# apcamargo/genomad

Hardware: AMD Instinct MI355X
Metric: 6 kbp windows classified/sec (higher is better)
Workload: dtype f16x3tk (conv2 read from a 137 GB table of all 14-mers in HBM - x2[t] is a function of the bases t-10 .. t+3 -, head A's pair products from an (entry, 9-mer) table, head A's y @ w_v rows from a 9-mer table, all exact f32; conv3 by Toom-Cook F(3,6) with split-f16 MFMA, 3 products per operand pair, f3

## Files before the change

genomad_amd/csrc/gnn_api.hip:

```cpp
#include <algorithm>
#include <map>
#include <mutex>
#include <cstdio>
#include <cmath>
#include <cstdlib>
#include <cstring>

#include "gnn_common.h"

namespace gnn {

static thread_local std::string g_last_error;
void set_error(const std::string& msg) { g_last_error = msg; }

bool debug_switch(const char* name) {
    static std::mutex mu;
    static std::map<std::string, bool> seen;
    std::lock_guard<std::mutex> lock(mu);
    auto it = seen.find(name);
    if (it != seen.end()) return it->second;
    const bool on = std::getenv(name) != nullptr;
    if (on)
        std::fprintf(stderr, "libgenomad_nn_hip: debug switch %s is set: NOT the production path (ordering or arithmetic may differ)\n", name);
    seen[name] = on;
    return on;
}

struct ProfScope {
    gnn_ctx* ctx;
    int id;
    hipEvent_t a = nullptr, b = nullptr;
    ProfScope(gnn_ctx* c, int kid) : ctx(c), id(kid) {
        if (!ctx->profile) return;
        auto take = [&]() {
            hipEvent_t e = nullptr;
            if (!ctx->event_pool.empty()) {
                e = ctx->event_pool.back();
                ctx->event_pool.pop_back();
            } else if (hipEventCreate(&e) != hipSuccess) {
                e = nullptr;
            }
            return e;
        };
        a = take();
        b = take();
        if (a) (void)hipEventRecord(a, ctx->stream);
    }
    ~ProfScope() {
        if (!ctx->profile || !a || !b) return;
        (void)hipEventRecord(b, ctx->stream);
        ctx->prof[id].pending.emplace_back(a, b);
    }
};

static void free_ws(Workspace& ws) { ws = Workspace(); }

constexpr size_t WS_BYTES_PER_WINDOW = ((size_t)2 * NPAIR + 2 * NP + (size_t)2 * POOLED * C + 4 * POOLED + FEAT) * sizeof(float);
constexpr int64_t MIN_CHUNK = 256;

static int ensure_ws(gnn_ctx* ctx, Workspace& ws, int64_t chunk, int64_t x_chunk) {
    if (ws.chunk < chunk || ws.x_chunk < x_chunk) {
        if (ctx->stream2) GNN_HIP(hipStreamSynchronize(ctx->stream2));
        ctx->back_pending[0] = ctx->back_pending[1] = false;
    }
    if (ws.chunk < chunk) {
        GNN_HIP(hipStreamSynchronize(ctx->stream));
        int rc = ws.mp.reserve((size_t)chunk * 2 * NPAIR);
        if (!rc) rc = ws.m.reserve((size_t)chunk * 2 * NP);
        if (!rc) rc = ws.yp.reserve((size_t)chunk * 2 * POOLED * C);
        if (!rc) rc = ws.logits.reserve((size_t)chunk * 2 * POOLED);
        if (!rc) rc = ws.alpha.reserve((size_t)chunk * 2 * POOLED);
        if (!rc) rc = ws.feat.reserve((size_t)chunk * FEAT);
        if (rc) {
            free_ws(ws);
            return rc;
        }
        ws.chunk = chunk;
    }
    if (ws.x_chunk < x_chunk) {
        GNN_HIP(hipStreamSynchronize(ctx->stream));
        ws.x_chunk = 0;
        for (DevBuf<float>& x : ws.x) x.reset();
        ws.tokens.reset();
        int rc = GNN_OK;
        for (DevBuf<float>& x : ws.x)
            if (!rc) rc = x.reserve((size_t)x_chunk * T * C);
        if (!rc) rc = ws.tokens.reserve((size_t)x_chunk * T);
        if (rc) {
            free_ws(ws);
            return rc;
        }
        ws.x_chunk = x_chunk;
    }
    return GNN_OK;
}

int flush_backend(gnn_ctx* ctx) {
    for (int i = 0; i < 2; ++i)
        if (ctx->back_pending[i]) {
            GNN_HIP(hipStreamWaitEvent(ctx->stream, ctx->ev_back[i], 0));
            ctx->back_pending[i] = false;
        }
    return GNN_OK;
}

int finish_pending(gnn_ctx* ctx) {
    if (ctx->back_pending[0] || ctx->back_pending[1]) {
        GNN_HIP(hipStreamSynchronize(ctx->stream2));
        ctx->back_pending[0] = ctx->back_pending[1] = false;
    }
    return GNN_OK;
}

static int check_ctx(gnn_ctx* ctx, bool flush = true) {
    if (!ctx) {
        set_error("ctx is NULL");
        return GNN_ERR_ARG;
    }
    GNN_HIP(hipSetDevice(ctx->device));
    if (!flush) return GNN_OK;
    static const bool event_wait = debug_switch("GNN_ASYNC_EVENT_WAIT");
// ... 141 lines not shown
    }
    bool overlap = allow_overlap && !f32 && ((chunk_overlap && n > chunk) || defer_last || pending);
    if (overlap && ctx->alt_failed_chunk > 0 && chunk >= ctx->alt_failed_chunk && ctx->ws_alt.chunk < chunk) {
        if ((rc = flush_backend(ctx))) return rc;
        overlap = false;
    }
    if (overlap && (rc = ensure_ws(ctx, ctx->ws_alt, chunk, 0)) == GNN_ERR_NOMEM) {
        std::fprintf(stderr, "libgenomad_nn_hip: no device memory for the second workspace of %lld windows: asynchronous calls run in order "
                     "(back end not overlapped) from here on\n", (long long)chunk);
        ctx->alt_failed_chunk = chunk;
        if ((rc = flush_backend(ctx))) return rc;
        overlap = false;
    } else if (rc) {
        return rc;
    }
    if (overlap) {
        if (!ctx->stream2) {
            GNN_HIP(hipStreamCreateWithFlags(&ctx->stream2, hipStreamNonBlocking));
            for (int i = 0; i < 2; ++i) {
                GNN_HIP(hipEventCreateWithFlags(&ctx->ev_front[i], hipEventDisableTiming));
                GNN_HIP(hipEventCreateWithFlags(&ctx->ev_back[i], hipEventDisableTiming));
            }
        }
    }
    struct StreamGuard {
        gnn_ctx* c;
        hipStream_t main;
        ~StreamGuard() { c->stream = main; }
    } guard{ctx, ctx->stream};
    for (int64_t a = 0; a < n; a += chunk) {
        const int64_t m = std::min(chunk, n - a);
        const uint8_t* b = bases_dev + a * W;
        if (!f32 && (reinterpret_cast<uintptr_t>(b) & 3u)) {
            if (ctx->align_buf.capacity() < (size_t)m * W) {
                GNN_HIP(hipStreamSynchronize(guard.main));
                if ((rc = ctx->align_buf.reserve((size_t)chunk * W))) return rc;
            }
            GNN_HIP(hipMemcpyAsync(ctx->align_buf, b, (size_t)m * W, hipMemcpyDeviceToDevice, guard.main));
            b = ctx->align_buf;
        }
        const int buf = ctx->buf_cur;
        if (overlap && ctx->back_pending[buf]) {
            GNN_HIP(hipStreamWaitEvent(guard.main, ctx->ev_back[buf], 0));
            ctx->back_pending[buf] = false;
        }
        static const bool poison = debug_switch("GNN_DEBUG_POISON");
        if (poison) {
            const Workspace& ws = ctx->ws;
            const size_t mm = (size_t)std::min<int64_t>(m, ws.chunk);
            auto fill = [&](float* p, size_t per_window) -> int {
                if (p && mm) GNN_HIP(hipMemsetAsync(p, 0xFF, mm * per_window * sizeof(float), guard.main));
                return GNN_OK;
            };
            if ((rc = fill(ws.mp, 2 * NPAIR)) || (rc = fill(ws.m, 2 * NP)) || (rc = fill(ws.yp, (size_t)2 * POOLED * C)) ||
                (rc = fill(ws.logits, 2 * POOLED)) || (rc = fill(ws.alpha, 2 * POOLED)) || (rc = fill(ws.feat, FEAT)))
                return rc;
            if (emb_dev)
                GNN_HIP(hipMemsetAsync(static_cast<uint8_t*>(emb_dev) + (size_t)a * HID * emb_elem_bytes(emb_dtype), 0xFF,
                                       (size_t)m * HID * emb_elem_bytes(emb_dtype), guard.main));
        }
        if (f32) {
            ProfScope ps(ctx, GNN_K_F32_FRONT);
            if ((rc = launch_front_f32(ctx, b, m))) return rc;
        } else {
            ProfScope ps(ctx, GNN_K_FUSED);
            rc = precision == GNN_PREC_F16X3TK ? launch_front_tk(ctx, b, m)
                 : precision == GNN_PREC_F16X3TC ? launch_front_tc(ctx, b, m)
                 : precision == GNN_PREC_F16C6 ? launch_front_c6(ctx, b, m)
                                               : launch_front_x3(ctx, b, m, precision);
            if (rc) return rc;
        }
        if (overlap) {
            GNN_HIP(hipEventRecord(ctx->ev_front[buf], guard.main));
            ctx->stream = ctx->stream2;
            GNN_HIP(hipStreamWaitEvent(ctx->stream2, ctx->ev_front[buf], 0));
        }
        {
            ProfScope ps(ctx, GNN_K_BACKEND);
            void* emb = emb_dev ? static_cast<uint8_t*>(emb_dev) + (size_t)a * HID * emb_elem_bytes(emb_dtype) : nullptr;
            rc = launch_backend(ctx, m, (precision == GNN_PREC_F16X3TC || precision == GNN_PREC_F16X3TK) ? GNN_PREC_F16X3 : precision,
                                scores_dev + a * GNN_CLASSES, emb, emb_dtype);
        }
        if (overlap) {
            if (!rc) {
                GNN_HIP(hipEventRecord(ctx->ev_back[buf], ctx->stream2));
                ctx->back_pending[buf] = true;
            }
            ctx->stream = guard.main;
            std::swap(ctx->ws, ctx->ws_alt);
            ctx->buf_cur ^= 1;
        }
        if (rc) return rc;
    }
    return defer_last ? GNN_OK : flush_backend(ctx);
}

}

using namespace gnn;

extern "C" {

const char* gnn_last_error(void) { return g_last_error.c_str(); }

int gnn_version(void) { return 300; }

int gnn_debug_pack_c6(const float* w, int k, int n, uint32_t* out, size_t out_words, size_t* need_words) {
// ... 500 lines not shown
    const size_t row = (size_t)HID * emb_elem_bytes(emb_dtype);
    if ((rc = ensure_stage(ctx, slab))) return rc;
    if (ctx->stage_emb.capacity() * sizeof(float) < (size_t)slab * row) {
        GNN_HIP(hipStreamSynchronize(ctx->stream));
        if ((rc = ctx->stage_emb.reserve((size_t)slab * HID))) return rc;
    }
    for (int64_t a0 = 0; a0 < n && !rc; a0 += slab) {
        const int64_t m = std::min(slab, n - a0);
        rc = stage_upload(ctx, bases_host + a0 * W, (size_t)m * W);
        if (!rc) rc = classify_chunks(ctx, ctx->stage_bases, m, precision, ctx->stage_scores, false, ctx->stage_emb, emb_dtype);
        if (!rc) {
            if (scores_host)
                GNN_HIP(hipMemcpyAsync(ctx->stage_scores_host, ctx->stage_scores, (size_t)m * GNN_CLASSES * sizeof(float),
                                       hipMemcpyDeviceToHost, ctx->stream));
            GNN_HIP(hipMemcpyAsync(static_cast<uint8_t*>(emb_host) + (size_t)a0 * row, ctx->stage_emb, (size_t)m * row,
                                   hipMemcpyDeviceToHost, ctx->stream));
            GNN_HIP(hipStreamSynchronize(ctx->stream));
            if (scores_host)
                std::memcpy(scores_host + a0 * GNN_CLASSES, ctx->stage_scores_host, (size_t)m * GNN_CLASSES * sizeof(float));
        }
    }
    return rc;
}

int gnn_classify(gnn_ctx* ctx, const uint8_t* bases_host, int64_t n, int precision, float* scores_host) {
    return gnn_debug_forward(ctx, bases_host, n, precision, scores_host, nullptr);
}

int gnn_debug_forward(gnn_ctx* ctx, const uint8_t* bases_host, int64_t n, int precision,
                      float* scores_host, const gnn_taps* taps) {
    int rc = check_ctx(ctx);
    if (rc) return rc;
    if (n < 0 || (n > 0 && (!bases_host || !scores_host))) {
        set_error("bad argument to gnn_classify");
        return GNN_ERR_ARG;
    }
    if (n == 0) return GNN_OK;
    if (taps) {
        const int64_t lim = precision == GNN_PREC_F32 ? ctx->chunk_f32 : ctx->chunk_fused;
        if (n > lim) {
            set_error("gnn_debug_forward with taps: n_windows exceeds one chunk (" + std::to_string(lim) + ")");
            return GNN_ERR_ARG;
        }
        if ((taps->x1 || taps->x2 || taps->x3) && precision != GNN_PREC_F32) {
            set_error("x1/x2/x3 taps exist only on the f32 path (the fused path keeps them in LDS)");
            return GNN_ERR_ARG;
        }
    }
    const int64_t slab = std::min<int64_t>(n, STAGE_MAX_WINDOWS);
    if ((rc = ensure_stage(ctx, slab))) return rc;
    for (int64_t a0 = 0; a0 < n && !rc; a0 += slab) {
        const int64_t m = std::min(slab, n - a0);
        rc = stage_upload(ctx, bases_host + a0 * W, (size_t)m * W);
        if (!rc) rc = classify_chunks(ctx, ctx->stage_bases, m, precision, ctx->stage_scores);
        if (!rc) {
            GNN_HIP(hipMemcpyAsync(ctx->stage_scores_host, ctx->stage_scores, (size_t)m * GNN_CLASSES * sizeof(float),
                                   hipMemcpyDeviceToHost, ctx->stream));
            GNN_HIP(hipStreamSynchronize(ctx->stream));
            std::memcpy(scores_host + a0 * GNN_CLASSES, ctx->stage_scores_host, (size_t)m * GNN_CLASSES * sizeof(float));
        }
    }
    if (!rc && taps && precision != GNN_PREC_F32 && n > ctx->chunk_fused) {
        set_error("gnn_debug_forward with taps: the launch size was reduced to " + std::to_string(ctx->chunk_fused) +
                  " windows for lack of device memory; the taps of " + std::to_string(n) + " windows do not fit one launch");
        return GNN_ERR_STATE;
    }
    if (!rc && taps) {
        const Workspace& ws = ctx->ws;
        auto out = [&](float* dst, const float* src, size_t count) {
            if (dst && !rc) rc = gnn_memcpy_d2h(ctx, dst, src, count * sizeof(float));
        };
        out(taps->x1, ws.x[0], (size_t)n * T * C);
        out(taps->x2, ws.x[1], (size_t)n * T * C);
        out(taps->x3, ws.x[2], (size_t)n * T * C);
        out(taps->feat, ws.feat, (size_t)n * FEAT);
        auto out2 = [&](float* dst_a, float* dst_b, const float* src, size_t per) {
            if ((!dst_a && !dst_b) || rc) return;
            std::vector<float> tmp((size_t)n * 2 * per);
            rc = gnn_memcpy_d2h(ctx, tmp.data(), src, tmp.size() * sizeof(float));
            if (rc) return;
            for (int64_t i = 0; i < n; ++i) {
                if (dst_a) std::memcpy(dst_a + i * per, tmp.data() + (i * 2 + 0) * per, per * sizeof(float));
                if (dst_b) std::memcpy(dst_b + i * per, tmp.data() + (i * 2 + 1) * per, per * sizeof(float));
            }
        };
        out2(taps->yp_a, taps->yp_b, ws.yp, (size_t)POOLED * C);
        out2(taps->alpha_a, taps->alpha_b, ws.alpha, (size_t)POOLED);
        out2(taps->m_a, taps->m_b, ws.m, (size_t)NP);
    }
    return rc;
}

static int upload_spans(gnn_ctx* ctx, const int64_t* starts_host, const int32_t* lens_host, int64_t n,
                        DevBuf<int64_t>& starts_dev, DevBuf<int32_t>& lens_dev) {
    for (int64_t i = 0; i < n; ++i)
        if (starts_host[i] < 0 || lens_host[i] < 0 || lens_host[i] > W) {
            set_error("span " + std::to_string(i) + " has a negative start or a length outside [0, 6000]");
            return GNN_ERR_ARG;
        }
    int rc = starts_dev.reserve((size_t)n);
    if (!rc) rc = lens_dev.reserve((size_t)n);
    if (!rc) rc = gnn_memcpy_h2d(ctx, starts_dev, starts_host, (size_t)n * sizeof(int64_t));
    if (!rc) rc = gnn_memcpy_h2d(ctx, lens_dev, lens_host, (size_t)n * sizeof(int32_t));
    return rc;
}

int gnn_span_byte_count(gnn_ctx* ctx, const uint8_t* seq_dev, const int64_t* starts_host, const int32_t* lens_host,
// ... 130 lines not shown
```

genomad_amd/csrc/gnn_backend.hip:

```cpp
#include <cstdlib>

#include "gnn_common.h"

namespace gnn {

__global__ __launch_bounds__(256) void m_kernel(const float* __restrict__ mp, const float* __restrict__ w_bias0,
                                                const float* __restrict__ w_bias1,
                                                const int32_t* __restrict__ slot0,
                                                const int32_t* __restrict__ slot1, float* __restrict__ m) {
    __shared__ float s[NPAIR];
    const int wi = blockIdx.x, h = blockIdx.y;
    const float* w_bias = h ? w_bias1 : w_bias0;
    const int32_t* slot = h ? slot1 : slot0;
    const float4* src = reinterpret_cast<const float4*>(mp + ((size_t)wi * 2 + h) * NPAIR);
    for (int i = threadIdx.x; i < NPAIR / 4; i += 256) reinterpret_cast<float4*>(s)[i] = src[i];
    __syncthreads();
    for (int p = threadIdx.x; p < NP; p += 256) {
        const int4 sl = reinterpret_cast<const int4*>(slot)[p];
        m[((size_t)wi * 2 + h) * NP + p] = w_bias[p] + s[sl.x] + s[sl.y] + s[sl.z] + s[sl.w];
    }
}

constexpr int LW = 64, LQ = 128, LK = 16;

__global__ __launch_bounds__(256) void logits_kernel(const float* __restrict__ m,
                                                     const float* __restrict__ w_qk0,
                                                     const float* __restrict__ w_qk1, int n,
                                                     float* __restrict__ logits) {
    __shared__ __attribute__((aligned(16))) float ms[LK][LW + 4];
    __shared__ __attribute__((aligned(16))) float qs[LK][LQ];
    const int h = blockIdx.z;
    const float* w_qk = h ? w_qk1 : w_qk0;
    const int w0 = blockIdx.y * LW;
    const int q0 = blockIdx.x * LQ;
    const int tw = threadIdx.x >> 4;
    const int tq = threadIdx.x & 15;
    float acc[4][8];
#pragma unroll
    for (int i = 0; i < 4; ++i)
#pragma unroll
        for (int k = 0; k < 8; ++k) acc[i][k] = 0.f;
    for (int p0 = 0; p0 < NP; p0 += LK) {
        {
            const int w = threadIdx.x >> 2, pq = (threadIdx.x & 3) * 4;
            float4 v = make_float4(0.f, 0.f, 0.f, 0.f);
            if (w0 + w < n && p0 + pq < NP)
                v = *reinterpret_cast<const float4*>(m + ((size_t)(w0 + w) * 2 + h) * NP + p0 + pq);
            ms[pq][w] = v.x;
            ms[pq + 1][w] = v.y;
            ms[pq + 2][w] = v.z;
            ms[pq + 3][w] = v.w;
        }
        for (int i = threadIdx.x; i < LK * LQ; i += 256) {
            const int q = i % LQ, p = i / LQ;
            qs[p][q] = (p0 + p < NP && q0 + q < POOLED) ? w_qk[(size_t)(p0 + p) * POOLED + q0 + q] : 0.f;
        }
        __syncthreads();
#pragma unroll 4
        for (int p = 0; p < LK; ++p) {
            const float4 a = *reinterpret_cast<const float4*>(&ms[p][tw * 4]);
            const float4 b0 = *reinterpret_cast<const float4*>(&qs[p][tq * 4]);
            const float4 b1 = *reinterpret_cast<const float4*>(&qs[p][64 + tq * 4]);
            const float av[4] = {a.x, a.y, a.z, a.w};
            const float bv[8] = {b0.x, b0.y, b0.z, b0.w, b1.x, b1.y, b1.z, b1.w};
#pragma unroll
            for (int i = 0; i < 4; ++i)
#pragma unroll
                for (int k = 0; k < 8; ++k) acc[i][k] = fmaf(av[i], bv[k], acc[i][k]);
        }
        __syncthreads();
    }
#pragma unroll
    for (int i = 0; i < 4; ++i) {
        const int w = w0 + tw * 4 + i;
        if (w >= n) continue;
#pragma unroll
        for (int k = 0; k < 8; ++k) {
            const int q = q0 + (k >> 2) * 64 + tq * 4 + (k & 3);
            if (q < POOLED) logits[((size_t)w * 2 + h) * POOLED + q] = acc[i][k];
        }
    }
}

typedef __bf16 bf16x8 __attribute__((ext_vector_type(8)));
typedef float f32x16 __attribute__((ext_vector_type(16)));

struct QkA {
    float4 v[2][2];
};
struct QkB {
    uint4 v[2][2];
};

__device__ __forceinline__ void qk_load(QkA& a, QkB& b, const float* __restrict__ mrow0, const float* __restrict__ mrow1,
                                        const uint4* __restrict__ bfrag, int ks, int lane) {
    const int k = ks * 16 + (lane >> 5) * 8;
    const float* rows[2] = {mrow0, mrow1};
#pragma unroll
    for (int mb = 0; mb < 2; ++mb) {
        if (k + 8 <= NP) {
            a.v[mb][0] = *reinterpret_cast<const float4*>(rows[mb] + k);
            a.v[mb][1] = *reinterpret_cast<const float4*>(rows[mb] + k + 4);
        } else {
            float t[8];
#pragma unroll
            for (int e = 0; e < 8; ++e) t[e] = k + e < NP ? rows[mb][k + e] : 0.f;
            a.v[mb][0] = make_float4(t[0], t[1], t[2], t[3]);
            a.v[mb][1] = make_float4(t[4], t[5], t[6], t[7]);
        }
    }
    const uint4* bp = bfrag + (size_t)ks * (QK_NBLK * 2 * 64);
#pragma unroll
    for (int nb = 0; nb < 2; ++nb) {
        b.v[nb][0] = bp[nb * 2 * 64];
        b.v[nb][1] = bp[nb * 2 * 64 + 64];
    }
}

template <int PASSES, bool F16>
__device__ __forceinline__ void qk_mfma(const QkA& a, const QkB& b, f32x16 (&acc)[2][2]) {
    typedef float f32x8 __attribute__((ext_vector_type(8)));
    typedef _Float16 f16x8q __attribute__((ext_vector_type(8)));
#pragma unroll
    for (int mb = 0; mb < 2; ++mb) {
        const f32x8 x = {a.v[mb][0].x, a.v[mb][0].y, a.v[mb][0].z, a.v[mb][0].w,
                         a.v[mb][1].x, a.v[mb][1].y, a.v[mb][1].z, a.v[mb][1].w};
        if constexpr (F16) {
            const f16x8q ah = __builtin_convertvector(x, f16x8q);
            const f16x8q al = __builtin_convertvector(x - __builtin_convertvector(ah, f32x8), f16x8q);
#pragma unroll
            for (int nb = 0; nb < 2; ++nb) {
                const f16x8q bh = __builtin_bit_cast(f16x8q, b.v[nb][0]);
                if constexpr (PASSES == 3) {
                    const f16x8q bl = __builtin_bit_cast(f16x8q, b.v[nb][1]);
                    acc[mb][nb] = __builtin_amdgcn_mfma_f32_32x32x16_f16(ah, bl, acc[mb][nb], 0, 0, 0);
                    acc[mb][nb] = __builtin_amdgcn_mfma_f32_32x32x16_f16(al, bh, acc[mb][nb], 0, 0, 0);
                }
                acc[mb][nb] = __builtin_amdgcn_mfma_f32_32x32x16_f16(ah, bh, acc[mb][nb], 0, 0, 0);
            }
        } else {
            const bf16x8 ah = __builtin_convertvector(x, bf16x8);
            const bf16x8 al = __builtin_convertvector(x - __builtin_convertvector(ah, f32x8), bf16x8);
#pragma unroll
            for (int nb = 0; nb < 2; ++nb) {
                const bf16x8 bh = __builtin_bit_cast(bf16x8, b.v[nb][0]);
                if constexpr (PASSES == 3) {
                    const bf16x8 bl = __builtin_bit_cast(bf16x8, b.v[nb][1]);
                    acc[mb][nb] = __builtin_amdgcn_mfma_f32_32x32x16_bf16(ah, bl, acc[mb][nb], 0, 0, 0);
                    acc[mb][nb] = __builtin_amdgcn_mfma_f32_32x32x16_bf16(al, bh, acc[mb][nb], 0, 0, 0);
                }
                acc[mb][nb] = __builtin_amdgcn_mfma_f32_32x32x16_bf16(ah, bh, acc[mb][nb], 0, 0, 0);
            }
        }
    }
}

template <int PASSES, bool F16 = false>
__global__ __launch_bounds__(256) void logits_mfma_kernel(const float* __restrict__ m, const uint4* __restrict__ frag0,
                                                          const uint4* __restrict__ frag1, int n,
                                                          float* __restrict__ logits) {
    const int lane = threadIdx.x & 63, wave = threadIdx.x >> 6;
    const int h = blockIdx.z;
    const int w0 = blockIdx.y * 64;
    const int nb0 = blockIdx.x * 8 + wave * 2;
    const uint4* bfrag = (h ? frag1 : frag0) + (size_t)nb0 * 2 * 64 + lane;
    const float* mrow0 = m + ((size_t)min(w0 + (lane & 31), n - 1) * 2 + h) * NP;
    const float* mrow1 = m + ((size_t)min(w0 + 32 + (lane & 31), n - 1) * 2 + h) * NP;
    f32x16 acc[2][2];
#pragma unroll
    for (int i = 0; i < 2; ++i)
#pragma unroll
        for (int j = 0; j < 2; ++j)
#pragma unroll
            for (int r = 0; r < 16; ++r) acc[i][j][r] = 0.f;
    QkA a0, a1;
    QkB b0, b1;
    qk_load(a0, b0, mrow0, mrow1, bfrag, 0, lane);
#pragma unroll 1
    for (int ks = 0; ks < QK_KSTEPS; ks += 2) {
        qk_load(a1, b1, mrow0, mrow1, bfrag, ks + 1, lane);
        qk_mfma<PASSES, F16>(a0, b0, acc);
        qk_load(a0, b0, mrow0, mrow1, bfrag, min(ks + 2, QK_KSTEPS - 1), lane);
        qk_mfma<PASSES, F16>(a1, b1, acc);
    }
#pragma unroll
    for (int mb = 0; mb < 2; ++mb)
#pragma unroll
        for (int r = 0; r < 16; ++r) {
            const int w = w0 + mb * 32 + (r & 3) + 8 * (r >> 2) + 4 * (lane >> 5);
            if (w >= n) continue;
#pragma unroll
            for (int nb = 0; nb < 2; ++nb) {
                const int q = (nb0 + nb) * 32 + (lane & 31);
                if (q < POOLED) logits[((size_t)w * 2 + h) * POOLED + q] = acc[mb][nb][r];
            }
        }
}

__global__ __launch_bounds__(256) void attn_kernel(const float* __restrict__ logits,
                                                   const float* __restrict__ yp,
                                                   float* __restrict__ alpha_out,
                                                   float* __restrict__ feat) {
    __shared__ float a[POOLED + 3];
    __shared__ float red[256];
    const int wi = blockIdx.x, h = blockIdx.y;
    const float* lg = logits + ((size_t)wi * 2 + h) * POOLED;
    float mx = -INFINITY;
    for (int q = threadIdx.x; q < POOLED; q += 256) {
        const float v = lg[q];
        a[q] = v;
        mx = fmaxf(mx, v);
    }
    red[threadIdx.x] = mx;
    __syncthreads();
    for (int s = 128; s > 0; s >>= 1) {
        if (threadIdx.x < s) red[threadIdx.x] = fmaxf(red[threadIdx.x], red[threadIdx.x + s]);
        __syncthreads();
    }
    mx = red[0];
    __syncthreads();
    float sum = 0.f;
    for (int q = threadIdx.x; q < POOLED; q += 256) {
        const float e = expf(a[q] - mx);
        a[q] = e;
        sum += e;
    }
    red[threadIdx.x] = sum;
    __syncthreads();
    for (int s = 128; s > 0; s >>= 1) {
        if (threadIdx.x < s) red[threadIdx.x] += red[threadIdx.x + s];
        __syncthreads();
    }
    const float inv = 1.f / red[0];
    __syncthreads();
    for (int q = threadIdx.x; q < POOLED; q += 256) {
        const float v = a[q] * inv;
        a[q] = v;
        alpha_out[((size_t)wi * 2 + h) * POOLED + q] = v;
    }
    __syncthreads();
    const int cq = threadIdx.x & 31, g = threadIdx.x >> 5;
    const float4* y = reinterpret_cast<const float4*>(yp + ((size_t)wi * 2 + h) * POOLED * C) + cq;
    float4 acc = make_float4(0.f, 0.f, 0.f, 0.f);
    int q = g;
    for (; q + 24 < POOLED; q += 32) {
        typedef float ntf4 __attribute__((ext_vector_type(4)));
        const ntf4* yn = reinterpret_cast<const ntf4*>(y);
        const ntf4 v0 = __builtin_nontemporal_load(yn + (size_t)q * (C / 4)), v1 = __builtin_nontemporal_load(yn + (size_t)(q + 8) * (C / 4)),
                   v2 = __builtin_nontemporal_load(yn + (size_t)(q + 16) * (C / 4)), v3 = __builtin_nontemporal_load(yn + (size_t)(q + 24) * (C / 4));
        const float a0 = a[q], a1 = a[q + 8], a2 = a[q + 16], a3 = a[q + 24];
        acc.x = fmaf(a0, v0.x, acc.x); acc.y = fmaf(a0, v0.y, acc.y); acc.z = fmaf(a0, v0.z, acc.z); acc.w = fmaf(a0, v0.w, acc.w);
        acc.x = fmaf(a1, v1.x, acc.x); acc.y = fmaf(a1, v1.y, acc.y); acc.z = fmaf(a1, v1.z, acc.z); acc.w = fmaf(a1, v1.w, acc.w);
        acc.x = fmaf(a2, v2.x, acc.x); acc.y = fmaf(a2, v2.y, acc.y); acc.z = fmaf(a2, v2.z, acc.z); acc.w = fmaf(a2, v2.w, acc.w);
        acc.x = fmaf(a3, v3.x, acc.x); acc.y = fmaf(a3, v3.y, acc.y); acc.z = fmaf(a3, v3.z, acc.z); acc.w = fmaf(a3, v3.w, acc.w);
    }
    for (; q < POOLED; q += 8) {
        const float4 v = y[(size_t)q * (C / 4)];
        const float aq = a[q];
        acc.x = fmaf(aq, v.x, acc.x); acc.y = fmaf(aq, v.y, acc.y); acc.z = fmaf(aq, v.z, acc.z); acc.w = fmaf(aq, v.w, acc.w);
    }
    __shared__ float4 part[8][32];
    part[g][cq] = acc;
    __syncthreads();
    if (threadIdx.x < 128) {
        const int c = threadIdx.x;
        float s = 0.f;
#pragma unroll
        for (int k = 0; k < 8; ++k) s += reinterpret_cast<const float*>(&part[k][c >> 2])[c & 3];
        feat[(size_t)wi * FEAT + h * C + c] = s;
    }
}

constexpr int DW = 8;

__device__ __forceinline__ uint16_t f32_to_bf16_rne(float v) {
    const uint32_t u = __float_as_uint(v);
    if ((u & 0x7fffffffu) > 0x7f800000u) return (uint16_t)((u >> 16) | 0x0040u);
    return (uint16_t)((u + 0x7fffu + ((u >> 16) & 1u)) >> 16);
}

template <int EMB>
__global__ __launch_bounds__(512) void dense_kernel(const float* __restrict__ feat,
                                                    const float* __restrict__ d1k, const float* __restrict__ d1b,
                                                    const float* __restrict__ d2k, const float* __restrict__ d2b,
                                                    const float* __restrict__ d3k, const float* __restrict__ d3b,
                                                    int n, float* __restrict__ scores, void* __restrict__ emb) {
    __shared__ float f[DW][FEAT];
    __shared__ float h1[DW][HID];
    __shared__ float h2[DW][HID];
    __shared__ float lg[DW][4];
    const int w0 = blockIdx.x * DW;
// ... 108 lines not shown
                const int row = mb * 32 + (r & 3) + 8 * (r >> 2) + 4 * (lane >> 5);
                const float v = acc[mb][nb][r] + b;
                hs[row * DM_STRIDE + col] = v < 0.f ? 0.f : v;
            }
    }
}

__global__ __launch_bounds__(256) void dense_mfma_kernel(const float* __restrict__ feat, const uint4* __restrict__ f1,
                                                         const float* __restrict__ d1b, const uint4* __restrict__ f2,
                                                         const float* __restrict__ d2b, const float* __restrict__ d3k,
                                                         const float* __restrict__ d3b, int n, float* __restrict__ scores) {
    __shared__ __attribute__((aligned(16))) float hs[DM_ROWS * DM_STRIDE];
    __shared__ float lg[DM_ROWS][4];
    const int lane = threadIdx.x & 63, wave = threadIdx.x >> 6;
    const int w0 = blockIdx.x * DM_ROWS;
    f32x16 acc[DM_MB][4];
    static_assert(DM_MB == 1, "the first layer's row clamp is written for one 32-window block per workgroup");
    dense_mfma_layer<FEAT / 16, false>(feat + (size_t)min(w0 + (lane & 31), n - 1) * FEAT, 32 * FEAT, f1, wave, lane, acc);
    dense_mfma_store(hs, d1b, wave, lane, acc);
    __syncthreads();
    dense_mfma_layer<HID / 16, true>(hs + (lane & 31) * DM_STRIDE, 32 * DM_STRIDE, f2, wave, lane, acc);
    __syncthreads();
    dense_mfma_store(hs, d2b, wave, lane, acc);
    __syncthreads();
    for (int o = wave; o < DM_ROWS * GNN_CLASSES; o += 4) {
        const int w = o / GNN_CLASSES, cl = o % GNN_CLASSES;
        float s = 0.f;
        for (int k = lane; k < HID; k += 64) s = fmaf(hs[w * DM_STRIDE + k], d3k[(size_t)k * GNN_CLASSES + cl], s);
#pragma unroll
        for (int off = 32; off >= 1; off >>= 1) s += __shfl_xor(s, off, 64);
        if (lane == 0) lg[w][cl] = s + d3b[cl];
    }
    __syncthreads();
    const int j = threadIdx.x;
    if (j < DM_ROWS && w0 + j < n) {
        const float a = lg[j][0], b = lg[j][1], c = lg[j][2];
        const float mx = fmaxf(a, fmaxf(b, c));
        const float ea = expf(a - mx), eb = expf(b - mx), ec = expf(c - mx);
        const float inv = 1.f / (ea + eb + ec);
        float* o = scores + (size_t)(w0 + j) * GNN_CLASSES;
        o[0] = ea * inv;
        o[1] = eb * inv;
        o[2] = ec * inv;
    }
}

int launch_backend(gnn_ctx* ctx, int64_t n, int precision, float* scores_dev, void* emb_dev, int emb_dtype) {
    if (emb_dev && (precision == GNN_PREC_F16C6 || precision == GNN_PREC_F16C8 || (emb_dtype != GNN_EMB_F32 && emb_dtype != GNN_EMB_BF16))) {
        set_error("embeddings: the dense head of this arithmetic does not produce them (f16c6 is frozen), or a bad gnn_emb_dtype");
        return GNN_ERR_ARG;
    }
    const DeviceWeights& d = ctx->w;
    Workspace& ws = ctx->ws;
    hipLaunchKernelGGL(m_kernel, dim3((unsigned)n, 2), dim3(256), 0, ctx->stream, ws.mp, d.w_bias[0], d.w_bias[1],
                       d.slot[0], d.slot[1], ws.m);
    static_assert(QK_KSTEPS % 2 == 0 && QK_NBLK % 8 == 0, "logits_mfma_kernel tiling");
    static const bool logits_f32 = debug_switch("GNN_LOGITS_F32");
    const dim3 qk_grid(QK_NBLK / 8, (unsigned)((n + 63) / 64), 2);
    const uint4* qf0 = reinterpret_cast<const uint4*>(d.wqk_frag[0]);
    const uint4* qf1 = reinterpret_cast<const uint4*>(d.wqk_frag[1]);
    if (precision == GNN_PREC_BF16X3 || precision == GNN_PREC_F16C8 || precision == GNN_PREC_F16C6)
        hipLaunchKernelGGL(logits_mfma_kernel<3>, qk_grid, dim3(256), 0, ctx->stream, ws.m, qf0, qf1, (int)n, ws.logits);
    else if (precision == GNN_PREC_BF16)
        hipLaunchKernelGGL(logits_mfma_kernel<1>, qk_grid, dim3(256), 0, ctx->stream, ws.m, qf0, qf1, (int)n, ws.logits);
    else if (precision == GNN_PREC_F16X3 && !logits_f32)
        hipLaunchKernelGGL((logits_mfma_kernel<3, true>), qk_grid, dim3(256), 0, ctx->stream, ws.m,
                           reinterpret_cast<const uint4*>(d.wqk_frag_h[0]), reinterpret_cast<const uint4*>(d.wqk_frag_h[1]), (int)n, ws.logits);
    else
        hipLaunchKernelGGL(logits_kernel, dim3((POOLED + LQ - 1) / LQ, (unsigned)((n + LW - 1) / LW), 2), dim3(256), 0,
                           ctx->stream, ws.m, d.w_qk[0], d.w_qk[1], (int)n, ws.logits);
    hipLaunchKernelGGL(attn_kernel, dim3((unsigned)n, 2), dim3(256), 0, ctx->stream, ws.logits, ws.yp, ws.alpha,
                       ws.feat);
    if (precision != GNN_PREC_F16C6 && precision != GNN_PREC_F16C8) {
        const dim3 grid((unsigned)((n + DW - 1) / DW));
        if (!emb_dev)
            hipLaunchKernelGGL(dense_kernel<0>, grid, dim3(512), 0, ctx->stream, ws.feat, d.d1_k, d.d1_b, d.d2_k, d.d2_b, d.d3_k,
                               d.d3_b, (int)n, scores_dev, nullptr);
        else if (emb_dtype == GNN_EMB_F32)
            hipLaunchKernelGGL(dense_kernel<GNN_EMB_F32 + 1>, grid, dim3(512), 0, ctx->stream, ws.feat, d.d1_k, d.d1_b, d.d2_k, d.d2_b,
                               d.d3_k, d.d3_b, (int)n, scores_dev, emb_dev);
        else
            hipLaunchKernelGGL(dense_kernel<GNN_EMB_BF16 + 1>, grid, dim3(512), 0, ctx->stream, ws.feat, d.d1_k, d.d1_b, d.d2_k, d.d2_b,
                               d.d3_k, d.d3_b, (int)n, scores_dev, emb_dev);
    } else {
        hipLaunchKernelGGL(dense_mfma_kernel, dim3((unsigned)((n + DM_ROWS - 1) / DM_ROWS)), dim3(256), 0, ctx->stream, ws.feat,
                           reinterpret_cast<const uint4*>(d.d1_frag), d.d1_b, reinterpret_cast<const uint4*>(d.d2_frag), d.d2_b,
                           d.d3_k, d.d3_b, (int)n, scores_dev);
    }
    GNN_HIP(hipGetLastError());
    return GNN_OK;
}

__global__ void segment_mean_kernel(const float* __restrict__ scores, const int64_t* __restrict__ ids,
                                    int64_t n, int64_t n_seg, float* __restrict__ out) {
    const int64_t i = (int64_t)blockIdx.x * blockDim.x + threadIdx.x;
    if (i >= n_seg * GNN_CLASSES) return;
    const int64_t seg = i / GNN_CLASSES;
    const int cl = (int)(i % GNN_CLASSES);
    int64_t lo = 0, hi = n;
    while (lo < hi) {
        const int64_t mid = (lo + hi) >> 1;
        if (ids[mid] < seg) lo = mid + 1; else hi = mid;
    }
    const int64_t a = lo;
    hi = n;
    while (lo < hi) {
        const int64_t mid = (lo + hi) >> 1;
        if (ids[mid] <= seg) lo = mid + 1; else hi = mid;
    }
    float s = 0.f;
    for (int64_t k = a; k < lo; ++k) s += scores[k * GNN_CLASSES + cl];
    out[i] = lo > a ? s / (float)(lo - a) : 0.f;
}

}

using namespace gnn;

extern "C" int gnn_segment_mean(gnn_ctx* ctx, const float* scores_host, const int64_t* ids_host, int64_t n,
                                int64_t n_segments, float* out_host) {
    if (!ctx || n < 0 || n_segments < 0 || (n > 0 && (!scores_host || !ids_host)) ||
        (n_segments > 0 && !out_host)) {
        set_error("bad argument to gnn_segment_mean");
        return GNN_ERR_ARG;
    }
// ... 37 lines not shown
```

genomad_amd/csrc/gnn_common.h:

```cpp
#pragma once
#include <hip/hip_runtime.h>
#include <stdint.h>
#include <string>
#include <vector>

#include "../../include/genomad_nn.h"
#include "gnn_devmem.h"

namespace gnn {

constexpr int W = GNN_WINDOW;
constexpr int T = GNN_TOKENS;
constexpr int C = GNN_CH;
constexpr int KS = GNN_KSIZE;
constexpr int NP = GNN_PATCHES;
constexpr int PS = GNN_PATCH_SIZE;
constexpr int NPAIR = NP * PS;
constexpr int POOLED = GNN_POOLED;
constexpr int FEAT = GNN_FEAT;
constexpr int HID = GNN_HIDDEN;
constexpr float LRELU = 0.1f;
constexpr float BN_EPS = 1e-3f;

constexpr int FT = 128;
// ... 21 lines not shown
    float* conv_b[2] = {nullptr, nullptr};
    float* weff_sorted[2] = {nullptr, nullptr};
    int32_t* pos_sorted[2] = {nullptr, nullptr};
    int32_t* slot[2] = {nullptr, nullptr};
    int32_t* bucket_ptr[2] = {nullptr, nullptr};
    float* conv1_pairs = nullptr;
    float* w_bias[2] = {nullptr, nullptr};
    float* w_qk[2] = {nullptr, nullptr};
    float* w_v[2] = {nullptr, nullptr};
    float* d1_k = nullptr;
    float* d1_b = nullptr;
    float* d2_k = nullptr;
    float* d2_b = nullptr;
    float* d3_k = nullptr;
    float* d3_b = nullptr;
    uint16_t* d1_frag = nullptr;
    uint16_t* d2_frag = nullptr;
    uint16_t* conv_frag[2] = {nullptr, nullptr};
    uint16_t* wv_frag[2] = {nullptr, nullptr};
    uint16_t* wqk_frag[2] = {nullptr, nullptr};
    uint16_t* wqk_frag_h[2] = {nullptr, nullptr};
    uint16_t* conv_frag_h[2] = {nullptr, nullptr};
    uint16_t* wv_frag_h[2] = {nullptr, nullptr};
    uint32_t* conv_c6[2] = {nullptr, nullptr};
    uint32_t* wv_c6[2] = {nullptr, nullptr};
    float* conv1_pairs6 = nullptr;
    float* weff6[2] = {nullptr, nullptr};
    int32_t* bucket_ptr6[2] = {nullptr, nullptr};
    DevBuf<float> c6_yp_const;
    DevBuf<float> c6_mp_const;
    uint16_t* tc_frag[2] = {nullptr, nullptr};
    float tc_inv_s[2] = {1.f, 1.f};
    int32_t* bucket_ptr96[2] = {nullptr, nullptr};
    DevBuf<float> tc_yp_const;
    DevBuf<float> tc_mp_const;
    DevBuf<float> tc_wva_tbl;
    DevBuf<float> tk_x2_tbl;
    DevBuf<float> tk_mpa_tbl;
    DevBuf<float> tk_x1t_tbl;
    DevBuf<float> tk_pt_tbl;
    DevBuf<float> tk_yp_const;
    DevBuf<float> tk_mp_const;
    DevBuf<float> x3_yp_const[2];
    DevBuf<float> x3_mp_const[2];
};

struct Workspace {
    int64_t chunk = 0;
    DevBuf<uint16_t> tokens;
    DevBuf<float> x[3];
    int64_t x_chunk = 0;
    DevBuf<float> mp;
    DevBuf<float> m;
    DevBuf<float> yp;
    DevBuf<float> logits;
    DevBuf<float> alpha;
    DevBuf<float> feat;
};

struct ContigWorkspace;

struct ProfileSlot {
    double total_ms = 0.0;
    int64_t launches = 0;
    std::vector<std::pair<hipEvent_t, hipEvent_t>> pending;
};

}

struct gnn_ctx {
    int device = 0;
    hipStream_t stream = nullptr;
    bool has_weights = false;
    gnn::DeviceWeights w;
    gnn::Workspace ws;
    gnn::Workspace ws_alt;
    hipStream_t stream2 = nullptr;
    hipEvent_t ev_front[2] = {nullptr, nullptr}, ev_back[2] = {nullptr, nullptr};
    bool back_pending[2] = {false, false};
    int buf_cur = 0;
    int64_t chunk_fused = 16384;
    int64_t alt_failed_chunk = 0;
    bool chunk_explicit = false;
    int64_t chunk_f32 = 64;
    bool profile = false;
    gnn::ProfileSlot prof[GNN_K_COUNT];
    std::vector<hipEvent_t> event_pool;
    std::vector<gnn::DevBuf<unsigned char>> owned;
    int cu_count = 0;
    int last_split = 1;
    bool time_split = true;
    bool c6_pad_skip = true;
    gnn::DevBuf<unsigned long long> phase_cycles;
    gnn::ContigWorkspace* contig_ws = nullptr;
    gnn::DevBuf<uint8_t> stage_bases;
    gnn::DevBuf<float> stage_emb;
    gnn::DevBuf<float> emb_scores;
    gnn::DevBuf<float> stage_scores;
    gnn::PinnedBuf<float> stage_scores_host;
    gnn::PinnedBuf<uint8_t> pin[2];
    hipEvent_t pin_ev[2] = {nullptr, nullptr};
    bool pin_busy[2] = {false, false};
    gnn::DevBuf<uint8_t> align_buf;
    void* comm = nullptr;
    int comm_ranks = 1, comm_rank = 0;
    gnn::DevBuf<unsigned char> comm_scratch;
};

namespace gnn {

template <typename Tp>
int upload(gnn_ctx* ctx, const Tp* host, size_t count, Tp** dev) {
    DevBuf<unsigned char> b;
    if (int rc = b.upload(reinterpret_cast<const unsigned char*>(host), count * sizeof(Tp))) return rc;
    *dev = reinterpret_cast<Tp*>(b.get());
    ctx->owned.emplace_back(std::move(b));
    return GNN_OK;
}
template <typename Tp>
int upload(gnn_ctx* ctx, const std::vector<Tp>& v, Tp** dev) {
    return upload(ctx, v.data(), v.size(), dev);
}

template <typename Run>
int all_n_consts(gnn_ctx* ctx, DevBuf<float>& yp, DevBuf<float>& mp, Run&& run) {
    DevBuf<uint8_t> bn;
    int rc = bn.reserve(W);
    if (!rc) rc = yp.reserve((size_t)2 * POOLED * C);
    if (!rc) rc = mp.reserve((size_t)2 * NPAIR);
    if (rc) return rc;
    hipError_t e = hipMemsetAsync(bn, 'N', W, ctx->stream);
    if (e == hipSuccess) {
        run(bn.get(), yp.get(), mp.get());
        e = hipGetLastError();
    }
    if (e == hipSuccess) e = hipStreamSynchronize(ctx->stream);
    if (e == hipSuccess) return GNN_OK;
// ... 45 lines not shown
```

Before: 318,100.

## Pre-split attention query into f16 hi/lo planes and stage through LDS in logits GEMM

m_kernel now writes the attention input already split into hi/lo f16 (or bf16) planes, padded to the GEMM K, and writes the f32 copy only when taps are requested. The logits MFMA kernel drops the per-step conversion and boundary handling and widens to 512 threads covering all N blocks per workgroup. It double-buffers the A operand through LDS, so it is read from global once per tile instead of once per N-block group. The alpha write in attn_kernel is skipped unless taps are requested. This adds a workspace buffer and more LDS and register use per block.

```diff
diff --git a/genomad_amd/csrc/gnn_api.hip b/genomad_amd/csrc/gnn_api.hip
--- a/genomad_amd/csrc/gnn_api.hip
+++ b/genomad_amd/csrc/gnn_api.hip
@@ -55,7 +55,7 @@
 
 static void free_ws(Workspace& ws) { ws = Workspace(); }
 
-constexpr size_t WS_BYTES_PER_WINDOW = ((size_t)2 * NPAIR + 2 * NP + (size_t)2 * POOLED * C + 4 * POOLED + FEAT) * sizeof(float);
+constexpr size_t WS_BYTES_PER_WINDOW = ((size_t)2 * NPAIR + 2 * NP + 2 * QK_KSTEPS * 16 + (size_t)2 * POOLED * C + 4 * POOLED + FEAT) * sizeof(float);
 constexpr int64_t MIN_CHUNK = 256;
 
 static int ensure_ws(gnn_ctx* ctx, Workspace& ws, int64_t chunk, int64_t x_chunk) {
@@ -67,6 +67,7 @@
         GNN_HIP(hipStreamSynchronize(ctx->stream));
         int rc = ws.mp.reserve((size_t)chunk * 2 * NPAIR);
         if (!rc) rc = ws.m.reserve((size_t)chunk * 2 * NP);
+        if (!rc) rc = ws.msplit.reserve((size_t)chunk * 2 * QK_KSTEPS * 16);
         if (!rc) rc = ws.yp.reserve((size_t)chunk * 2 * POOLED * C);
         if (!rc) rc = ws.logits.reserve((size_t)chunk * 2 * POOLED);
         if (!rc) rc = ws.alpha.reserve((size_t)chunk * 2 * POOLED);
@@ -314,7 +315,7 @@
                 if (p && mm) GNN_HIP(hipMemsetAsync(p, 0xFF, mm * per_window * sizeof(float), guard.main));
                 return GNN_OK;
             };
-            if ((rc = fill(ws.mp, 2 * NPAIR)) || (rc = fill(ws.m, 2 * NP)) || (rc = fill(ws.yp, (size_t)2 * POOLED * C)) ||
+            if ((rc = fill(ws.mp, 2 * NPAIR)) || (rc = fill(ws.m, 2 * NP)) || (rc = fill(reinterpret_cast<float*>(ws.msplit.get()), 2 * QK_KSTEPS * 16)) || (rc = fill(ws.yp, (size_t)2 * POOLED * C)) ||
                 (rc = fill(ws.logits, 2 * POOLED)) || (rc = fill(ws.alpha, 2 * POOLED)) || (rc = fill(ws.feat, FEAT)))
                 return rc;
             if (emb_dev)
@@ -921,7 +922,9 @@
     for (int64_t a0 = 0; a0 < n && !rc; a0 += slab) {
         const int64_t m = std::min(slab, n - a0);
         rc = stage_upload(ctx, bases_host + a0 * W, (size_t)m * W);
+        ctx->keep_taps = taps != nullptr;
         if (!rc) rc = classify_chunks(ctx, ctx->stage_bases, m, precision, ctx->stage_scores);
+        ctx->keep_taps = false;
         if (!rc) {
             GNN_HIP(hipMemcpyAsync(ctx->stage_scores_host, ctx->stage_scores, (size_t)m * GNN_CLASSES * sizeof(float),
                                    hipMemcpyDeviceToHost, ctx->stream));
diff --git a/genomad_amd/csrc/gnn_backend.hip b/genomad_amd/csrc/gnn_backend.hip
--- a/genomad_amd/csrc/gnn_backend.hip
+++ b/genomad_amd/csrc/gnn_backend.hip
@@ -4,20 +4,53 @@
 
 namespace gnn {
 
+constexpr int QK_KPAD = QK_KSTEPS * 16;
+constexpr int QK_ROW16 = QK_KSTEPS * 4;
+
+template <bool F32OUT, int SPLIT>
 __global__ __launch_bounds__(256) void m_kernel(const float* __restrict__ mp, const float* __restrict__ w_bias0,
                                                 const float* __restrict__ w_bias1,
                                                 const int32_t* __restrict__ slot0,
-                                                const int32_t* __restrict__ slot1, float* __restrict__ m) {
+                                                const int32_t* __restrict__ slot1, float* __restrict__ m,
+                                                uint4* __restrict__ msplit) {
     __shared__ float s[NPAIR];
+    __shared__ __attribute__((aligned(16))) float mo[SPLIT ? QK_KPAD : 1];
     const int wi = blockIdx.x, h = blockIdx.y;
     const float* w_bias = h ? w_bias1 : w_bias0;
     const int32_t* slot = h ? slot1 : slot0;
     const float4* src = reinterpret_cast<const float4*>(mp + ((size_t)wi * 2 + h) * NPAIR);
     for (int i = threadIdx.x; i < NPAIR / 4; i += 256) reinterpret_cast<float4*>(s)[i] = src[i];
     __syncthreads();
-    for (int p = threadIdx.x; p < NP; p += 256) {
-        const int4 sl = reinterpret_cast<const int4*>(slot)[p];
-        m[((size_t)wi * 2 + h) * NP + p] = w_bias[p] + s[sl.x] + s[sl.y] + s[sl.z] + s[sl.w];
+    for (int p = threadIdx.x; p < (SPLIT ? QK_KPAD : NP); p += 256) {
+        float v = 0.f;
+        if (p < NP) {
+            const int4 sl = reinterpret_cast<const int4*>(slot)[p];
+            v = w_bias[p] + s[sl.x] + s[sl.y] + s[sl.z] + s[sl.w];
+            if constexpr (F32OUT) m[((size_t)wi * 2 + h) * NP + p] = v;
+        }
+        if constexpr (SPLIT != 0) mo[p] = v;
+    }
+    if constexpr (SPLIT != 0) {
+        typedef float f32x8 __attribute__((ext_vector_type(8)));
+        typedef _Float16 f16x8 __attribute__((ext_vector_type(8)));
+        typedef __bf16 bf16x8m __attribute__((ext_vector_type(8)));
+        __syncthreads();
+        uint4* dst = msplit + ((size_t)wi * 2 + h) * QK_ROW16;
+        for (int g = threadIdx.x; g < QK_KPAD / 8; g += 256) {
+            const float4 x0 = *reinterpret_cast<const float4*>(mo + g * 8), x1 = *reinterpret_cast<const float4*>(mo + g * 8 + 4);
+            const f32x8 x = {x0.x, x0.y, x0.z, x0.w, x1.x, x1.y, x1.z, x1.w};
+            if constexpr (SPLIT == 2) {
+                const f16x8 hi = __builtin_convertvector(x, f16x8);
+                const f16x8 lo = __builtin_convertvector(x - __builtin_convertvector(hi, f32x8), f16x8);
+                dst[g * 2] = __builtin_bit_cast(uint4, hi);
+                dst[g * 2 + 1] = __builtin_bit_cast(uint4, lo);
+            } else {
+                const bf16x8m hi = __builtin_convertvector(x, bf16x8m);
+                const bf16x8m lo = __builtin_convertvector(x - __builtin_convertvector(hi, f32x8), bf16x8m);
+                dst[g * 2] = __builtin_bit_cast(uint4, hi);
+                dst[g * 2 + 1] = __builtin_bit_cast(uint4, lo);
+            }
+        }
     }
 }
 
@@ -85,51 +118,38 @@
 typedef __bf16 bf16x8 __attribute__((ext_vector_type(8)));
 typedef float f32x16 __attribute__((ext_vector_type(16)));
 
-struct QkA {
-    float4 v[2][2];
+constexpr int QA_KC = 6;
+constexpr int QA_STAGES = QK_KSTEPS / QA_KC;
+constexpr int QA_STAGE16 = QA_KC * 2 * 2 * 64;
+constexpr int QA_NB = QK_NBLK / 8;
+static_assert(QK_KSTEPS % QA_KC == 0 && QA_KC % 2 == 0 && QK_NBLK % 8 == 0 && QA_STAGE16 == 3 * 512, "logits_mfma_kernel tiling");
+
+struct QkB {
+    uint4 v[QA_NB][2];
 };
-struct QkB {
-    uint4 v[2][2];
-};
-
-__device__ __forceinline__ void qk_load(QkA& a, QkB& b, const float* __restrict__ mrow0, const float* __restrict__ mrow1,
-                                        const uint4* __restrict__ bfrag, int ks, int lane) {
-    const int k = ks * 16 + (lane >> 5) * 8;
-    const float* rows[2] = {mrow0, mrow1};
+
+template <int PASSES>
+__device__ __forceinline__ void qk_load_b(QkB& b, const uint4* __restrict__ bfrag, int ks) {
+    const uint4* bp = bfrag + (size_t)ks * (QK_NBLK * 2 * 64);
+#pragma unroll
+    for (int nb = 0; nb < QA_NB; ++nb) {
+        b.v[nb][0] = bp[nb * 2 * 64];
+        if constexpr (PASSES == 3) b.v[nb][1] = bp[nb * 2 * 64 + 64];
+    }
+}
+
+template <int PASSES, bool F16>
+__device__ __forceinline__ void qk_mfma(const uint4* __restrict__ a_ks, int lane, const QkB& b, f32x16 (&acc)[2][QA_NB]) {
+    typedef _Float16 f16x8q __attribute__((ext_vector_type(8)));
 #pragma unroll
     for (int mb = 0; mb < 2; ++mb) {
-        if (k + 8 <= NP) {
-            a.v[mb][0] = *reinterpret_cast<const float4*>(rows[mb] + k);
-            a.v[mb][1] = *reinterpret_cast<const float4*>(rows[mb] + k + 4);
-        } else {
-            float t[8];
-#pragma unroll
-            for (int e = 0; e < 8; ++e) t[e] = k + e < NP ? rows[mb][k + e] : 0.f;
-            a.v[mb][0] = make_float4(t[0], t[1], t[2], t[3]);
-            a.v[mb][1] = make_float4(t[4], t[5], t[6], t[7]);
-        }
-    }
-    const uint4* bp = bfrag + (size_t)ks * (QK_NBLK * 2 * 64);
-#pragma unroll
-    for (int nb = 0; nb < 2; ++nb) {
-        b.v[nb][0] = bp[nb * 2 * 64];
-        b.v[nb][1] = bp[nb * 2 * 64 + 64];
-    }
-}
-
-template <int PASSES, bool F16>
-__device__ __forceinline__ void qk_mfma(const QkA& a, const QkB& b, f32x16 (&acc)[2][2]) {
-    typedef float f32x8 __attribute__((ext_vector_type(8)));
-    typedef _Float16 f16x8q __attribute__((ext_vector_type(8)));
-#pragma unroll
-    for (int mb = 0; mb < 2; ++mb) {
-        const f32x8 x = {a.v[mb][0].x, a.v[mb][0].y, a.v[mb][0].z, a.v[mb][0].w,
-                         a.v[mb][1].x, a.v[mb][1].y, a.v[mb][1].z, a.v[mb][1].w};
+        const uint4 ahu = a_ks[(mb * 2 + 0) * 64 + lane];
+        uint4 alu = ahu;
+        if constexpr (PASSES == 3) alu = a_ks[(mb * 2 + 1) * 64 + lane];
         if constexpr (F16) {
-            const f16x8q ah = __builtin_convertvector(x, f16x8q);
-            const f16x8q al = __builtin_convertvector(x - __builtin_convertvector(ah, f32x8), f16x8q);
-#pragma unroll
-            for (int nb = 0; nb < 2; ++nb) {
+            const f16x8q ah = __builtin_bit_cast(f16x8q, ahu), al = __builtin_bit_cast(f16x8q, alu);
+#pragma unroll
+            for (int nb = 0; nb < QA_NB; ++nb) {
                 const f16x8q bh = __builtin_bit_cast(f16x8q, b.v[nb][0]);
                 if constexpr (PASSES == 3) {
                     const f16x8q bl = __builtin_bit_cast(f16x8q, b.v[nb][1]);
@@ -139,10 +159,9 @@
                 acc[mb][nb] = __builtin_amdgcn_mfma_f32_32x32x16_f16(ah, bh, acc[mb][nb], 0, 0, 0);
             }
         } else {
-            const bf16x8 ah = __builtin_convertvector(x, bf16x8);
-            const bf16x8 al = __builtin_convertvector(x - __builtin_convertvector(ah, f32x8), bf16x8);
-#pragma unroll
-            for (int nb = 0; nb < 2; ++nb) {
+            const bf16x8 ah = __builtin_bit_cast(bf16x8, ahu), al = __builtin_bit_cast(bf16x8, alu);
+#pragma unroll
+            for (int nb = 0; nb < QA_NB; ++nb) {
                 const bf16x8 bh = __builtin_bit_cast(bf16x8, b.v[nb][0]);
                 if constexpr (PASSES == 3) {
                     const bf16x8 bl = __builtin_bit_cast(bf16x8, b.v[nb][1]);
@@ -156,32 +175,56 @@
 }
 
 template <int PASSES, bool F16 = false>
-__global__ __launch_bounds__(256) void logits_mfma_kernel(const float* __restrict__ m, const uint4* __restrict__ frag0,
+__global__ __launch_bounds__(512) void logits_mfma_kernel(const uint4* __restrict__ msplit, const uint4* __restrict__ frag0,
                                                           const uint4* __restrict__ frag1, int n,
                                                           float* __restrict__ logits) {
+    __shared__ uint4 as[2][QA_STAGE16];
     const int lane = threadIdx.x & 63, wave = threadIdx.x >> 6;
-    const int h = blockIdx.z;
-    const int w0 = blockIdx.y * 64;
-    const int nb0 = blockIdx.x * 8 + wave * 2;
+    const int h = blockIdx.y;
+    const int w0 = blockIdx.x * 64;
+    const int nb0 = wave * QA_NB;
     const uint4* bfrag = (h ? frag1 : frag0) + (size_t)nb0 * 2 * 64 + lane;
-    const float* mrow0 = m + ((size_t)min(w0 + (lane & 31), n - 1) * 2 + h) * NP;
-    const float* mrow1 = m + ((size_t)min(w0 + 32 + (lane & 31), n - 1) * 2 + h) * NP;
-    f32x16 acc[2][2];
+    const uint4* arow = msplit + ((size_t)min(w0 + lane, n - 1) * 2 + h) * QK_ROW16 + wave;
+    int sdst[3];
+#pragma unroll
+    for (int j = 0; j < 3; ++j) {
+        const int pc = wave + 8 * j, ksl = pc >> 2, half = (pc >> 1) & 1, plane = pc & 1;
+        sdst[j] = ((ksl * 2 + (lane >> 5)) * 2 + plane) * 64 + half * 32 + (lane & 31);
+    }
+    f32x16 acc[2][QA_NB];
 #pragma unroll
     for (int i = 0; i < 2; ++i)
 #pragma unroll
-        for (int j = 0; j < 2; ++j)
+        for (int j = 0; j < QA_NB; ++j)
 #pragma unroll
             for (int r = 0; r < 16; ++r) acc[i][j][r] = 0.f;
-    QkA a0, a1;
+    uint4 st[3];
+#pragma unroll
+    for (int j = 0; j < 3; ++j) as[0][sdst[j]] = arow[8 * j];
     QkB b0, b1;
-    qk_load(a0, b0, mrow0, mrow1, bfrag, 0, lane);
+    qk_load_b<PASSES>(b0, bfrag, 0);
+    __syncthreads();
 #pragma unroll 1
-    for (int ks = 0; ks < QK_KSTEPS; ks += 2) {
-        qk_load(a1, b1, mrow0, mrow1, bfrag, ks + 1, lane);
-        qk_mfma<PASSES, F16>(a0, b0, acc);
-        qk_load(a0, b0, mrow0, mrow1, bfrag, min(ks + 2, QK_KSTEPS - 1), lane);
-        qk_mfma<PASSES, F16>(a1, b1, acc);
+    for (int c = 0; c < QA_STAGES; ++c) {
+        const bool more = c + 1 < QA_STAGES;
+        if (more) {
+#pragma unroll
+            for (int j = 0; j < 3; ++j) st[j] = arow[(c + 1) * (QA_KC * 4) + 8 * j];
+        }
+        const uint4* a_st = as[c & 1];
+#pragma unroll
+        for (int ksl = 0; ksl < QA_KC; ksl += 2) {
+            const int ks = c * QA_KC + ksl;
+            qk_load_b<PASSES>(b1, bfrag, ks + 1);
+            qk_mfma<PASSES, F16>(a_st + ksl * 256, lane, b0, acc);
+            qk_load_b<PASSES>(b0, bfrag, min(ks + 2, QK_KSTEPS - 1));
+            qk_mfma<PASSES, F16>(a_st + (ksl + 1) * 256, lane, b1, acc);
+        }
+        if (more) {
+#pragma unroll
+            for (int j = 0; j < 3; ++j) as[(c + 1) & 1][sdst[j]] = st[j];
+        }
+        __syncthreads();
     }
 #pragma unroll
     for (int mb = 0; mb < 2; ++mb)
@@ -190,13 +233,14 @@
             const int w = w0 + mb * 32 + (r & 3) + 8 * (r >> 2) + 4 * (lane >> 5);
             if (w >= n) continue;
 #pragma unroll
-            for (int nb = 0; nb < 2; ++nb) {
+            for (int nb = 0; nb < QA_NB; ++nb) {
                 const int q = (nb0 + nb) * 32 + (lane & 31);
                 if (q < POOLED) logits[((size_t)w * 2 + h) * POOLED + q] = acc[mb][nb][r];
             }
         }
 }
 
+template <bool ALPHA>
 __global__ __launch_bounds__(256) void attn_kernel(const float* __restrict__ logits,
                                                    const float* __restrict__ yp,
                                                    float* __restrict__ alpha_out,
@@ -236,7 +280,7 @@
     for (int q = threadIdx.x; q < POOLED; q += 256) {
         const float v = a[q] * inv;
         a[q] = v;
-        alpha_out[((size_t)wi * 2 + h) * POOLED + q] = v;
+        if constexpr (ALPHA) alpha_out[((size_t)wi * 2 + h) * POOLED + q] = v;
     }
     __syncthreads();
     const int cq = threadIdx.x & 31, g = threadIdx.x >> 5;
@@ -451,25 +495,38 @@
     }
     const DeviceWeights& d = ctx->w;
     Workspace& ws = ctx->ws;
-    hipLaunchKernelGGL(m_kernel, dim3((unsigned)n, 2), dim3(256), 0, ctx->stream, ws.mp, d.w_bias[0], d.w_bias[1],
-                       d.slot[0], d.slot[1], ws.m);
-    static_assert(QK_KSTEPS % 2 == 0 && QK_NBLK % 8 == 0, "logits_mfma_kernel tiling");
     static const bool logits_f32 = debug_switch("GNN_LOGITS_F32");
-    const dim3 qk_grid(QK_NBLK / 8, (unsigned)((n + 63) / 64), 2);
+    const bool taps = ctx->keep_taps;
+    const bool gemm_f32 = precision == GNN_PREC_F32 || (precision == GNN_PREC_F16X3 && logits_f32);
+    const bool gemm_f16 = precision == GNN_PREC_F16X3;
+    const dim3 m_grid((unsigned)n, 2);
+    uint4* msplit = reinterpret_cast<uint4*>(ws.msplit.get());
+#define GNN_M_KERNEL(F32OUT, SPLIT)                                                                                          \
+    hipLaunchKernelGGL((m_kernel<F32OUT, SPLIT>), m_grid, dim3(256), 0, ctx->stream, ws.mp, d.w_bias[0], d.w_bias[1], d.slot[0], \
+                       d.slot[1], ws.m, msplit)
+    if (gemm_f32) GNN_M_KERNEL(true, 0);
+    else if (gemm_f16 && taps) GNN_M_KERNEL(true, 2);
+    else if (gemm_f16) GNN_M_KERNEL(false, 2);
+    else if (taps) GNN_M_KERNEL(true, 1);
+    else GNN_M_KERNEL(false, 1);
+#undef GNN_M_KERNEL
+    const dim3 qk_grid((unsigned)((n + 63) / 64), 2);
     const uint4* qf0 = reinterpret_cast<const uint4*>(d.wqk_frag[0]);
     const uint4* qf1 = reinterpret_cast<const uint4*>(d.wqk_frag[1]);
-    if (precision == GNN_PREC_BF16X3 || precision == GNN_PREC_F16C8 || precision == GNN_PREC_F16C6)
-        hipLaunchKernelGGL(logits_mfma_kernel<3>, qk_grid, dim3(256), 0, ctx->stream, ws.m, qf0, qf1, (int)n, ws.logits);
-    else if (precision == GNN_PREC_BF16)
-        hipLaunchKernelGGL(logits_mfma_kernel<1>, qk_grid, dim3(256), 0, ctx->stream, ws.m, qf0, qf1, (int)n, ws.logits);
-    else if (precision == GNN_PREC_F16X3 && !logits_f32)
-        hipLaunchKernelGGL((logits_mfma_kernel<3, true>), qk_grid, dim3(256), 0, ctx->stream, ws.m,
-                           reinterpret_cast<const uint4*>(d.wqk_frag_h[0]), reinterpret_cast<const uint4*>(d.wqk_frag_h[1]), (int)n, ws.logits);
-    else
+    if (gemm_f32)
         hipLaunchKernelGGL(logits_kernel, dim3((POOLED + LQ - 1) / LQ, (unsigned)((n + LW - 1) / LW), 2), dim3(256), 0,
                            ctx->stream, ws.m, d.w_qk[0], d.w_qk[1], (int)n, ws.logits);
-    hipLaunchKernelGGL(attn_kernel, dim3((unsigned)n, 2), dim3(256), 0, ctx->stream, ws.logits, ws.yp, ws.alpha,
-                       ws.feat);
+    else if (gemm_f16)
+        hipLaunchKernelGGL((logits_mfma_kernel<3, true>), qk_grid, dim3(512), 0, ctx->stream, msplit,
+                           reinterpret_cast<const uint4*>(d.wqk_frag_h[0]), reinterpret_cast<const uint4*>(d.wqk_frag_h[1]), (int)n, ws.logits);
+    else if (precision == GNN_PREC_BF16)
+        hipLaunchKernelGGL(logits_mfma_kernel<1>, qk_grid, dim3(512), 0, ctx->stream, msplit, qf0, qf1, (int)n, ws.logits);
+    else
+        hipLaunchKernelGGL(logits_mfma_kernel<3>, qk_grid, dim3(512), 0, ctx->stream, msplit, qf0, qf1, (int)n, ws.logits);
+    if (taps)
+        hipLaunchKernelGGL(attn_kernel<true>, dim3((unsigned)n, 2), dim3(256), 0, ctx->stream, ws.logits, ws.yp, ws.alpha, ws.feat);
+    else
+        hipLaunchKernelGGL(attn_kernel<false>, dim3((unsigned)n, 2), dim3(256), 0, ctx->stream, ws.logits, ws.yp, ws.alpha, ws.feat);
     if (precision != GNN_PREC_F16C6 && precision != GNN_PREC_F16C8) {
         const dim3 grid((unsigned)((n + DW - 1) / DW));
         if (!emb_dev)
diff --git a/genomad_amd/csrc/gnn_common.h b/genomad_amd/csrc/gnn_common.h
--- a/genomad_amd/csrc/gnn_common.h
+++ b/genomad_amd/csrc/gnn_common.h
@@ -97,6 +97,7 @@
     int64_t x_chunk = 0;
     DevBuf<float> mp;
     DevBuf<float> m;
+    DevBuf<uint32_t> msplit;
     DevBuf<float> yp;
     DevBuf<float> logits;
     DevBuf<float> alpha;
@@ -128,6 +129,7 @@
     int64_t alt_failed_chunk = 0;
     bool chunk_explicit = false;
     int64_t chunk_f32 = 64;
+    bool keep_taps = false;
     bool profile = false;
     gnn::ProfileSlot prof[GNN_K_COUNT];
     std::vector<hipEvent_t> event_pool;
```

New measurement: 321,200 (median of 6 runs). Within noise of the previous version (+1.0%).
